# oscarknagg/voicemap

Measured on AMD Instinct MI355X. Metric: audio-sec/s embedded, 3s@16kHz siamese batch (training step), higher is better.
Workload: dtype f16; 1 GPU; siamese cfg-A train step (filters 128, embed 64, contrastive loss), 128 pairs/GPU of 3 s @ 16 kHz decimated x4 (L=12000), Adam(clipnorm 1), f16 storage; global_pairs=128, parallelism=dp1

## Files before the change

voicemap_amd/csrc/conv_common.hpp:

```cpp
#pragma once
#include <string.h>

#include <type_traits>

#include "common.hpp"

namespace vm {

constexpr int BM = 128, BN = 128;

template <int KB>
struct Geo {
    static constexpr int PITCH = KB + 16;
    static constexpr int TILE = BM * PITCH;
    static constexpr int CH = KB / 16;
    static constexpr int NCHUNK = BM * CH / 256;
};
constexpr int OUT_PITCH = BN * 4 + 16;

template <typename T> struct Mfma;
template <> struct Mfma<bf16> {
    static constexpr int KSTEP_BYTES = 32;
    using Frag = bf16x8;
    __device__ static inline Frag load(const char* row_ptr, int s, int kh) {
        return *reinterpret_cast<const Frag*>(row_ptr + (s * 2 + kh) * 16);
    }
    __device__ static inline f32x16 run(Frag a, Frag b, f32x16 c) {
        return __builtin_amdgcn_mfma_f32_32x32x16_bf16(a, b, c, 0, 0, 0);
    }
};
template <> struct Mfma<f16> {
    static constexpr int KSTEP_BYTES = 32;
    using Frag = f16x8;
    __device__ static inline Frag load(const char* row_ptr, int s, int kh) {
        return *reinterpret_cast<const Frag*>(row_ptr + (s * 2 + kh) * 16);
    }
    __device__ static inline f32x16 run(Frag a, Frag b, f32x16 c) {
        return __builtin_amdgcn_mfma_f32_32x32x16_f16(a, b, c, 0, 0, 0);
    }
};
template <> struct Mfma<float> {
    static constexpr int KSTEP_BYTES = 8;
    using Frag = float;
    __device__ static inline Frag load(const char* row_ptr, int s, int kh) {
        return *reinterpret_cast<const float*>(row_ptr + (s * 2 + kh) * 4);
    }
    __device__ static inline f32x16 run(Frag a, Frag b, f32x16 c) {
        return __builtin_amdgcn_mfma_f32_32x32x2f32(a, b, c, 0, 0, 0);
    }
};

template <typename T>
__device__ inline typename Mfma<T>::Frag ones16() {
    static_assert(sizeof(T) == 2, "16-bit storage types only");
    const uint32_t w = std::is_same<T, bf16>::value ? 0x3F803F80u : 0x3C003C00u;
    const u32x4 v = {w, w, w, w};
    return __builtin_bit_cast(typename Mfma<T>::Frag, v);
}

template <typename T> struct Mfma4;
template <> struct Mfma4<f16> {
// ... 159 lines not shown
```

voicemap_amd/csrc/conv_gemm.hip:

```cpp
#include "conv_common.hpp"

#ifndef VM_ABL
#define VM_ABL 0
#endif

namespace vm {

template <int KB>
constexpr int nt_lds_bytes() {
    return (2 * 2 * Geo<KB>::TILE > BM * OUT_PITCH + 4096) ? 2 * 2 * Geo<KB>::TILE : BM * OUT_PITCH + 4096;
}

template <typename T, int EPI, int KB, bool SPLIT = false>
__global__ __launch_bounds__(256) void conv_nt_kernel(NtArgs<T> p, int64_t n_groups) {
    static_assert(!SPLIT || (sizeof(T) == 4 && KB == 128), "split-bf16 arithmetic: fp32 storage, 128-byte slices");
    using G = Geo<KB>;
    constexpr int VEC = Elem<T>::kVec;
    constexpr int BK = KB / (int)sizeof(T);
    __shared__ __attribute__((aligned(16))) char lds[nt_lds_bytes<KB>()];

    const int tid = threadIdx.x, lane = tid & 63, w = tid >> 6, wm = w >> 1, wn = w & 1;
    const int nk = (p.Ktot + BK - 1) / BK;

    int lds_off[G::NCHUNK], kch[G::NCHUNK], srow[G::NCHUNK];
// ... 358 lines not shown
            issue(0);
            for (int kt = 0; kt < nk; ++kt) {
                __syncthreads();
                if (kt + 1 < nk) issue(kt + 1);
                const char* bufbase = lds + (kt & 1) * 2 * OPB;
                mma_slice_swz<T, KB>(bufbase, bufbase + OPB, wm, wn, lane, acc);
            }

            nt_epilogue<T, EPI>(p, lds, acc, n, tl, t0, n0, tid, lane, w, wm, wn);
            __syncthreads();
        }
    }
}

namespace n2 {
constexpr int TM = 256, TN = 128, KB = 64, RING = 3;
constexpr int A_BYTES = TM * KB, B_BYTES = TN * KB, STAGE = A_BYTES + B_BYTES;
constexpr int TP = TN * 2 + 16;
constexpr int LDS_BYTES = (RING * STAGE > TM * TP) ? RING * STAGE : TM * TP;
static_assert(2 * LDS_BYTES <= 160 * 1024, "two workgroups per CU");
}

template <typename T, int EPI>
__device__ inline void n2_load_bias(const NtArgs<T>& p, f32x4 (&b4)[2][4], int c0) {
#pragma unroll
    for (int j = 0; j < 2; ++j)
#pragma unroll
        for (int g = 0; g < 4; ++g) {
            b4[j][g] = f32x4{0.f, 0.f, 0.f, 0.f};
            if (EPI != EPI_DGRAD) b4[j][g] = *reinterpret_cast<const f32x4*>(p.bias + c0 + 32 * j + 8 * g);
        }
}
template <typename T>
__device__ inline void n2_fold_edge(const NtArgs<T>& p, f32x16 (&acc)[4][2], int row, int which, int wm, int r, int c0) {
    if ((row >> 7) != wm) return;
    const float* hb = p.fold_hb + (which ? 2 * p.N : 0) + c0;
    f32x4 h[2][4];
#pragma unroll
    for (int j = 0; j < 2; ++j)
#pragma unroll
        for (int g = 0; g < 4; ++g) h[j][g] = *reinterpret_cast<const f32x4*>(hb + 32 * j + 8 * g);
    const int rw = row & 127;
#pragma unroll
    for (int i = 0; i < 4; ++i) {
#pragma unroll
        for (int j = 0; j < 2; ++j) {
            const float m = (32 * i + r == rw) ? 1.f : 0.f;
#pragma unroll
            for (int g = 0; g < 4; ++g)
#pragma unroll
                for (int e = 0; e < 4; ++e) acc[i][j][4 * g + e] -= m * h[j][g][e];
        }
    }
}
__device__ inline void n2_fill_acc(f32x16 (&acc)[4][2], const f32x4 (&b4)[2][4]) {
#pragma unroll
    for (int j = 0; j < 2; ++j)
#pragma unroll
        for (int g = 0; g < 4; ++g)
#pragma unroll
            for (int i = 0; i < 4; ++i)
#pragma unroll
                for (int e = 0; e < 4; ++e) acc[i][j][4 * g + e] = b4[j][g][e];
}
#if defined(VM_EXPERIMENT_PROFILE_EPI)
extern __device__ unsigned int g_prof[];
__device__ inline void vm_epi_mark(int k) {
    const long long t = __builtin_amdgcn_s_memtime();
    if ((threadIdx.x & 63) == 0 && blockIdx.x < 8192) g_prof[((int64_t)blockIdx.x * 4 + (threadIdx.x >> 6)) * 8 + k] = (unsigned int)t;
}
#if VM_EXPERIMENT_PROFILE_EPI + 0 == 2
#define VM_EPI_MARK(k)
#define VM_RED_MARK(k) vm_epi_mark(k)
#else
#define VM_EPI_MARK(k) vm_epi_mark(k)
#define VM_RED_MARK(k)
#endif
#else
#define VM_EPI_MARK(k)
#define VM_RED_MARK(k)
#endif
struct N2DrainSync {
    __device__ inline void sync() { __syncthreads(); }
    __device__ inline void point() {}
};

template <typename T, int EPI>
__device__ inline void n2_tile_write(const NtArgs<T>& p, char* lds, const f32x16 (&acc)[4][2], int t0, int n0, int trows, int lane, int wm, int wn,
                                     const f32x4 (&negc)[2][4]) {
    using namespace n2;
    const int r = lane & 31, kh = lane >> 5;
    constexpr bool FWD = EPI == EPI_FWD || EPI == EPI_FWD_FOLD;
    const bool red = EPI == EPI_DGRAD && p.red_a != nullptr;
    const int valid = (p.L - t0) < trows ? (p.L - t0) : trows;
    constexpr bool CAN_CENTRE = EPI == EPI_FWD_FOLD && std::is_same<T, f16>::value;
    const bool ctrd = CAN_CENTRE && p.fold_ctr != nullptr;
    auto body = [&](auto ctrd_c) {
        constexpr bool CTRD = decltype(ctrd_c)::value;
        uint32_t nc16[2][4][2];
        if constexpr (CTRD) {
            typedef _Float16 h2 __attribute__((ext_vector_type(2)));
#pragma unroll
            for (int j = 0; j < 2; ++j)
#pragma unroll
                for (int g = 0; g < 4; ++g) {
                    nc16[j][g][0] = __builtin_bit_cast(uint32_t, h2{(_Float16)negc[j][g][0], (_Float16)negc[j][g][1]});
                    nc16[j][g][1] = __builtin_bit_cast(uint32_t, h2{(_Float16)negc[j][g][2], (_Float16)negc[j][g][3]});
                }
        }
#pragma unroll
        for (int i = 0; i < 4; ++i) {
#pragma unroll
            for (int j = 0; j < 2; ++j) {
                const int mb = wm * 128 + i * 32;
                const int m = mb + r;
                const bool partial = mb + 32 > valid;
                const bool zero = (FWD || red) && partial && m >= valid;
#pragma unroll
                for (int g = 0; g < 4; ++g) {
                    const int nl = wn * 64 + j * 32 + 8 * g + 4 * kh;
                    T o[4];
#pragma unroll
                    for (int e = 0; e < 4; ++e) o[e] = Elem<T>::from_f(acc[i][j][4 * g + e]);
                    u32x2 pk = *reinterpret_cast<const u32x2*>(o);
                    if constexpr (CTRD) {
                        uint32_t lo = pk[0], hi = pk[1];
                        asm("v_pk_max_f16 %0, %1, %2" : "=v"(lo) : "v"(lo), "v"(nc16[j][g][0]));
                        asm("v_pk_max_f16 %0, %1, %2" : "=v"(hi) : "v"(hi), "v"(nc16[j][g][1]));
                        pk[0] = lo;
                        pk[1] = hi;
                    } else if constexpr (EPI != EPI_DGRAD) {
                        uint32_t lo = pk[0], hi = pk[1];
                        asm("v_pk_max_i16 %0, %1, 0" : "=v"(lo) : "v"(lo));
                        asm("v_pk_max_i16 %0, %1, 0" : "=v"(hi) : "v"(hi));
                        pk[0] = lo;
                        pk[1] = hi;
                    }
                    pk[0] = zero ? 0u : pk[0];
                    pk[1] = zero ? 0u : pk[1];
                    *reinterpret_cast<u32x2*>(lds + m * TP + nl * 2) = pk;
                }
            }
        }
    };
    if constexpr (CAN_CENTRE) {
        if (ctrd) body(std::true_type{});
        else body(std::false_type{});
    } else {
        body(std::false_type{});
    }
}

template <typename T, int EPI, typename BarT>
__device__ inline void n2_tile_drain(const NtArgs<T>& p, char* lds, int64_t n, int tl, int t0, int n0, int trows, int tid, int lane, int w,
                                     BarT& bar) {
    using namespace n2;
    using V8 = typename Mfma<T>::Frag;
    const int kh = lane >> 5;
    constexpr bool FWD = EPI == EPI_FWD || EPI == EPI_FWD_FOLD;
    const bool stats = FWD && p.stat_sum != nullptr && !(VM_ABL & 8);
    const bool red = EPI == EPI_DGRAD && p.red_a != nullptr;
    const int valid = (p.L - t0) < trows ? (p.L - t0) : trows;
    const int c8 = tid & 15, rg = tid >> 4;
    if (EPI == EPI_FWD_POOL) {
// ... 283 lines not shown
                d2[h][1] = Mfma4<T>::run(dhi[q], ahi[rs], d2[h][1]);
            }
        }
        const int cn = lane & 31;
        const int rows2 = 2 * p.tilesL;
#pragma unroll
        for (int h = 0; h < 2; ++h) {
            float ds = d1[h][0][0] + d1[h][1][0], dq = 0.f;
#pragma unroll
            for (int e = 0; e < 4; ++e) dq = e == (lane & 3) ? d2[h][0][e] + d2[h][1][e] : dq;
            ds += __shfl_xor(ds, 32, 64);
            dq += __shfl_xor(dq, 32, 64);
            const int64_t srow = n * rows2 + 2 * tl + h;
            if (kh == 0) {
                p.stat_sum[srow * p.N + n0 + 32 * w + cn] = ds;
                p.stat_sq[srow * p.N + n0 + 32 * w + cn] = dq;
            }
        }
    }
}


template <typename T, int EPI>
__device__ inline void n2_epilogue(const NtArgs<T>& p, char* lds, const f32x16 (&acc)[4][2], int64_t n, int tl, int t0, int n0, int trows,
                                   int tid, int lane, int w, int wm, int wn) {
    f32x4 negc[2][4];
    if constexpr (EPI == EPI_FWD_FOLD && std::is_same<T, f16>::value) {
        if (p.fold_ctr != nullptr) {
#pragma unroll
            for (int j = 0; j < 2; ++j)
#pragma unroll
                for (int g = 0; g < 4; ++g) {
                    const f32x4 c = *reinterpret_cast<const f32x4*>(p.fold_ctr + n0 + (wn * 64 + j * 32) + 8 * g + 4 * (lane >> 5));
                    negc[j][g] = f32x4{-c[0], -c[1], -c[2], -c[3]};
                }
        }
    }
    VM_EPI_MARK(1);
    __syncthreads();
    VM_EPI_MARK(2);
    n2_tile_write<T, EPI>(p, lds, acc, t0, n0, trows, lane, wm, wn, negc);
    VM_EPI_MARK(3);
    __syncthreads();
    VM_EPI_MARK(4);
    N2DrainSync bar;
    n2_tile_drain<T, EPI>(p, lds, n, tl, t0, n0, trows, tid, lane, w, bar);
}

namespace n2r {
constexpr int TROWS = 254;
constexpr int A_BLK = 256 * 64, B_STG = 128 * 64;
constexpr int B0 = 3 * A_BLK;
constexpr int OPER = 3 * A_BLK + 3 * B_STG;
static_assert(OPER <= n2::LDS_BYTES, "operand rings fit under the epilogue tile");
}

__device__ inline void wait_vm_0246(int n) {
    if (n >= 6) {
// ... 49 lines not shown
    int tn;
    {
        const unsigned v = blockIdx.x, tiles_n = (unsigned)p.tilesN;
        if ((n_groups & 7) == 0) {
            const unsigned j = v >> 3, q = j / tiles_n;
            tn = (int)(j - q * tiles_n);
            group = q * 8 + (v & 7);
        } else {
            group = v / tiles_n;
            tn = (int)(v - group * tiles_n);
        }
    }
    const unsigned nw = group / (unsigned)p.tilesL;
    const int tl = (int)(group - nw * (unsigned)p.tilesL);
    const int64_t n = nw;
    const int t0 = tl * TROWS, n0 = tn * TN;
    if (n2_pool_dead_tile<T, EPI>(p, n, t0, n0, tid)) return;
    if constexpr (EPI == EPI_FWD_FOLD) {
        const unsigned tw = nw / (unsigned)p.tower_windows;
        p.bt += tw * p.bt_tower_stride;
        p.fold_hb += tw * 4 * p.N;
        if (p.fold_ctr != nullptr) p.fold_ctr += tw * p.N;
    }
    f32x4 bias4[2][4];
    if constexpr (EPI == EPI_FWD_FOLD) p.bias = p.fold_hb + 3 * p.N;
    n2_load_bias<T, EPI>(p, bias4, n0 + wn * 64 + 4 * (lane >> 5));

    const int lrow = lane >> 2, lchunk = lane & 3;
    const char* a_src[4];
    const char* b_src[2];
#pragma unroll
    for (int i = 0; i < 4; ++i) {
        const int row = (w + 4 * i) * 16 + lrow;
        int pr = t0 + row;
        pr = pr < p.L + 2 ? pr : p.L + 1;
        a_src[i] = reinterpret_cast<const char*>(p.a + n * p.a_win_stride + (int64_t)pr * p.a_c) + ((lchunk ^ ((row >> 2) & 3)) << 4);
    }
#pragma unroll
    for (int i = 0; i < 2; ++i) {
        const int row = (w + 4 * i) * 16 + lrow;
        b_src[i] = reinterpret_cast<const char*>(p.bt + (int64_t)(n0 + row) * p.Ktot) + ((lchunk ^ ((row >> 2) & 3)) << 4);
    }
    auto issue_a = [&](int blk, int chunk, int i0) {
        char* base = lds + blk * A_BLK;
#pragma unroll
        for (int i = 0; i < 2; ++i) glds16(a_src[i0 + i] + chunk * KB, base + __builtin_amdgcn_readfirstlane((w + 4 * (i0 + i)) * 1024));
    };
    auto issue_b = [&](int stg, int ko) {
        char* base = lds + B0 + stg * B_STG;
#pragma unroll
        for (int i = 0; i < 2; ++i) glds16(b_src[i] + ko, base + __builtin_amdgcn_readfirstlane((w + 4 * i) * 1024));
    };

    const int r = lane & 31, kh = lane >> 5;
    int a_addr[3][2], b_addr[2];
#pragma unroll
    for (int tap = 0; tap < 3; ++tap) {
        const int row = wm * 128 + r + tap;
#pragma unroll
        for (int ks = 0; ks < 2; ++ks) a_addr[tap][ks] = row * KB + (((2 * ks + kh) ^ ((row >> 2) & 3)) << 4);
    }
    {
        const int row = wn * 64 + r;
#pragma unroll
        for (int ks = 0; ks < 2; ++ks) b_addr[ks] = B0 + row * KB + (((2 * ks + kh) ^ ((row >> 2) & 3)) << 4);
    }

#if defined(__HIP_DEVICE_COMPILE__)
    const uint32_t lds0 = (uint32_t)(uintptr_t)(__attribute__((address_space(3))) const char*)lds;
#else
    const uint32_t lds0 = 0;
#endif

    VM_PROF(const long long pt_s2 = __builtin_amdgcn_s_memtime();)
    issue_a(0, 0, 0);
    issue_a(0, 0, 2);
    issue_b(0, 0);
    if (chunks > 1) {
        issue_a(1, 1, 0);
        issue_a(1, 1, 2);
    }
    issue_b(1, row_bytes);
    VM_PROF(const long long pt_s3 = __builtin_amdgcn_s_memtime();)
    f32x16 acc[4][2];
    n2_fill_acc(acc, bias4);
    int n_wait = (chunks > 1 ? 4 : 0) + 2;
    int ia_prev = 0;
    int b_tap = 2, b_chunk_off = 0, b_stage = 2;
    int a_blk = 0, b_cur = 0;
    for (int c = 0; c < chunks; ++c) {
        const bool more_a = c + 2 < chunks;
        const int a_next_blk = a_blk == 0 ? 2 : a_blk - 1;
#pragma unroll
        for (int tap = 0; tap < 3; ++tap) {
            const int kt = 3 * c + tap;
            wait_vm_0246(n_wait);
            __builtin_amdgcn_s_barrier();
            VM_PROF(if (kt == 0) pt_bar = __builtin_amdgcn_s_memtime();)
            int ib = 0, ia = 0;
            {
                if (kt + 2 < nk && !(VM_ABL & 1)) {
                    issue_b(b_stage, b_tap * row_bytes + b_chunk_off);
                    b_stage = b_stage == 2 ? 0 : b_stage + 1;
                    if (++b_tap == 3) {
                        b_tap = 0;
                        b_chunk_off += KB;
                    }
                    ib = 2;
                }
                if (tap < 2 && more_a && !(VM_ABL & 2)) {
                    issue_a(a_next_blk, c + 2, 2 * tap);
                    ia = 2;
                }
            }
            n_wait = ia_prev + ib + ia;
            ia_prev = ia;
            const uint32_t aa0 = lds0 + a_blk * A_BLK + a_addr[tap][0], aa1 = lds0 + a_blk * A_BLK + a_addr[tap][1];
            const uint32_t bb0 = lds0 + b_cur * B_STG + b_addr[0], bb1 = lds0 + b_cur * B_STG + b_addr[1];
            b_cur = b_cur == 2 ? 0 : b_cur + 1;
            u32x4 a0[4], b0[2], a1[4], b1[2];
            asm volatile("ds_read_b128 %0, %1" : "=v"(b0[0]) : "v"(bb0));
            asm volatile("ds_read_b128 %0, %1" : "=v"(a0[0]) : "v"(aa0));
            asm volatile("ds_read_b128 %0, %1 offset:2048" : "=v"(b0[1]) : "v"(bb0));
            asm volatile("ds_read_b128 %0, %1 offset:2048" : "=v"(a0[1]) : "v"(aa0));
            asm volatile("ds_read_b128 %0, %1 offset:4096" : "=v"(a0[2]) : "v"(aa0));
            asm volatile("ds_read_b128 %0, %1 offset:6144" : "=v"(a0[3]) : "v"(aa0));
            asm volatile("ds_read_b128 %0, %1" : "=v"(b1[0]) : "v"(bb1));
            asm volatile("ds_read_b128 %0, %1 offset:2048" : "=v"(b1[1]) : "v"(bb1));
            asm volatile("ds_read_b128 %0, %1" : "=v"(a1[0]) : "v"(aa1));
            asm volatile("ds_read_b128 %0, %1 offset:2048" : "=v"(a1[1]) : "v"(aa1));
            asm volatile("ds_read_b128 %0, %1 offset:4096" : "=v"(a1[2]) : "v"(aa1));
            asm volatile("ds_read_b128 %0, %1 offset:6144" : "=v"(a1[3]) : "v"(aa1));
#define VM_MM(A, B, I, J) acc[I][J] = Mfma<T>::run(__builtin_bit_cast(V8, B), __builtin_bit_cast(V8, A), acc[I][J])
            __builtin_amdgcn_sched_barrier(0);
            asm volatile("s_waitcnt lgkmcnt(9)" : "+v"(b0[0]), "+v"(a0[0]), "+v"(b0[1]));
            VM_MM(a0[0], b0[0], 0, 0);
            VM_MM(a0[0], b0[1], 0, 1);
            __builtin_amdgcn_sched_barrier(0);
            asm volatile("s_waitcnt lgkmcnt(8)" : "+v"(a0[1]));
            VM_MM(a0[1], b0[0], 1, 0);
            VM_MM(a0[1], b0[1], 1, 1);
            __builtin_amdgcn_sched_barrier(0);
            asm volatile("s_waitcnt lgkmcnt(7)" : "+v"(a0[2]));
            VM_MM(a0[2], b0[0], 2, 0);
            VM_MM(a0[2], b0[1], 2, 1);
            __builtin_amdgcn_sched_barrier(0);
            asm volatile("s_waitcnt lgkmcnt(6)" : "+v"(a0[3]));
            VM_MM(a0[3], b0[0], 3, 0);
            VM_MM(a0[3], b0[1], 3, 1);
            __builtin_amdgcn_sched_barrier(0);
            asm volatile("s_waitcnt lgkmcnt(3)" : "+v"(b1[0]), "+v"(b1[1]), "+v"(a1[0]));
            VM_MM(a1[0], b1[0], 0, 0);
            VM_MM(a1[0], b1[1], 0, 1);
            __builtin_amdgcn_sched_barrier(0);
            asm volatile("s_waitcnt lgkmcnt(2)" : "+v"(a1[1]));
            VM_MM(a1[1], b1[0], 1, 0);
            VM_MM(a1[1], b1[1], 1, 1);
            __builtin_amdgcn_sched_barrier(0);
            asm volatile("s_waitcnt lgkmcnt(1)" : "+v"(a1[2]));
            VM_MM(a1[2], b1[0], 2, 0);
            VM_MM(a1[2], b1[1], 2, 1);
            __builtin_amdgcn_sched_barrier(0);
            asm volatile("s_waitcnt lgkmcnt(0)" : "+v"(a1[3]));
            VM_MM(a1[3], b1[0], 3, 0);
            VM_MM(a1[3], b1[1], 3, 1);
            __builtin_amdgcn_sched_barrier(0);
#undef VM_MM
            __builtin_amdgcn_sched_barrier(0);
            VM_PROF(if (kt == 0) pt_first = __builtin_amdgcn_s_memtime();)
        }
        a_blk = a_blk == 2 ? 0 : a_blk + 1;
    }
    VM_PROF(const long long pt_loop = __builtin_amdgcn_s_memtime();)
    if constexpr (EPI == EPI_FWD_FOLD) {
        const int c0 = n0 + wn * 64 + 4 * (lane >> 5), rl = p.L - 1 - t0;
        if (t0 == 0) n2_fold_edge<T>(p, acc, 0, 0, wm, lane & 31, c0);
        if (rl >= 0 && rl < TROWS) n2_fold_edge<T>(p, acc, rl, 1, wm, lane & 31, c0);
    }
    n2_epilogue<T, EPI>(p, lds, acc, n, tl, t0, n0, TROWS, tid, lane, w, wm, wn);
#if defined(VM_EXPERIMENT_PROFILE)
    {
        asm volatile("s_waitcnt vmcnt(0)" ::: "memory");
        const long long pt_end = __builtin_amdgcn_s_memtime();
        if (lane == 0 && blockIdx.x < 8192) {
            unsigned int* q = g_prof + ((int64_t)blockIdx.x * 4 + w) * 8;
            q[0] = (unsigned int)(pt_end - pt_start);
            q[1] = (unsigned int)(pt_first - pt_start);
            q[2] = (unsigned int)(pt_loop - pt_first);
            q[3] = (unsigned int)(pt_end - pt_loop);
            q[4] = (unsigned int)(pt_s2 - pt_start);
            q[5] = (unsigned int)(pt_s3 - pt_s2);
            q[6] = (unsigned int)(pt_bar - pt_s3);
            q[7] = (unsigned int)(pt_first - pt_bar);
        }
    }
#endif
}


#ifndef VM_NT3_ABL
// ... 70 lines not shown
    {
        const unsigned v = blockIdx.x, tiles_n = (unsigned)p.tilesN;
        if ((n_groups & 7) == 0) {
            const unsigned j = v >> 3, q = j / tiles_n;
            tn = (int)(j - q * tiles_n);
            group = q * 8 + (v & 7);
        } else {
            group = v / tiles_n;
            tn = (int)(v - group * tiles_n);
        }
    }
    const unsigned nw = group / (unsigned)p.tilesL;
    const int tl = (int)(group - nw * (unsigned)p.tilesL);
    const int64_t n = nw;
    const int t0 = tl * n2r::TROWS, n0 = tn * TN;
    if (n2_pool_dead_tile<T, EPI>(p, n, t0, n0, tid)) return;
    unsigned tw = 0;
    if constexpr (EPI == EPI_FWD_FOLD) {
        tw = nw / (unsigned)p.tower_windows;
        p.fold_hb += tw * 4 * p.N;
        if (p.fold_ctr != nullptr) p.fold_ctr += tw * p.N;
    }
    if constexpr (EPI == EPI_FWD_FOLD) p.bias = p.fold_hb + 3 * p.N;
    f32x4 bias_lo[2][4], bias_hi[2][4];
    if constexpr (EPI != EPI_DGRAD) {
        const float* bp = p.bias + n0 + wn * 64;
#pragma unroll
        for (int j = 0; j < 2; ++j)
#pragma unroll
            for (int g = 0; g < 4; ++g) {
                bias_lo[j][g] = *reinterpret_cast<const f32x4*>(bp + 32 * j + 8 * g);
                bias_hi[j][g] = *reinterpret_cast<const f32x4*>(bp + 32 * j + 8 * g + 4);
            }
    }

    const int lrow = lane >> 2, lchunk = lane & 3;
    const char* a_src[4];
#pragma unroll
    for (int i = 0; i < 4; ++i) {
        const int row = (w + 4 * i) * 16 + lrow;
        int pr = t0 + row;
        pr = pr < p.L + 2 ? pr : p.L + 1;
        a_src[i] = reinterpret_cast<const char*>(p.a + n * p.a_win_stride + (int64_t)pr * p.a_c) + ((lchunk ^ ((row >> 2) & 3)) << 4);
    }
    auto issue_a = [&](int blk, int chunk, int i0) {
        char* base = lds + blk * A_BLK;
#pragma unroll
        for (int i = 0; i < 2; ++i) glds16(a_src[i0 + i] + chunk * KB, base + __builtin_amdgcn_readfirstlane((w + 4 * (i0 + i)) * 1024));
    };
    auto issue_a1 = [&](int blk, int chunk, int i) {
        glds16(a_src[i] + chunk * KB, lds + blk * A_BLK + __builtin_amdgcn_readfirstlane((w + 4 * i) * 1024));
    };
    uint64_t bbase;
    {
        const uint64_t q = (uint64_t)(uintptr_t)p.bt_packed +
                           ((uint64_t)tw * (unsigned)(p.N >> 6) + (unsigned)((n0 >> 6) + wn)) * (uint64_t)(NK * n3::KT_BYTES);
        const uint32_t lo = __builtin_amdgcn_readfirstlane((uint32_t)q), hi = __builtin_amdgcn_readfirstlane((uint32_t)(q >> 32));
        bbase = ((uint64_t)hi << 32) | lo;
    }
    const uint32_t bvoff = lane * 16;
    u32x4 bs[3][4];
#define VM_LOAD_SET(KT)                                                           \
    {                                                                             \
        const uint64_t sb_ = bbase + (uint64_t)((KT) * n3::KT_BYTES);             \
        VM_GLOAD_FRAG(bs[(KT) % 3][0], bvoff, sb_, 0);                            \
        VM_GLOAD_FRAG(bs[(KT) % 3][1], bvoff, sb_, 1024);                         \
        VM_GLOAD_FRAG(bs[(KT) % 3][2], bvoff, sb_, 2048);                         \
        VM_GLOAD_FRAG(bs[(KT) % 3][3], bvoff, sb_, 3072);                         \
    }

    const int r = lane & 31, kh = lane >> 5;
    int a_addr[3][2];
#pragma unroll
    for (int tap = 0; tap < 3; ++tap) {
        const int row = wm * 128 + r + tap;
#pragma unroll
        for (int ks = 0; ks < 2; ++ks) a_addr[tap][ks] = row * KB + (((2 * ks + kh) ^ ((row >> 2) & 3)) << 4);
    }
#if defined(__HIP_DEVICE_COMPILE__)
    const uint32_t lds0 = (uint32_t)(uintptr_t)(__attribute__((address_space(3))) const char*)lds;
#else
    const uint32_t lds0 = 0;
#endif

    VM_PROF(const long long pt_s2 = __builtin_amdgcn_s_memtime();)
    issue_a(0, 0, 0);
    issue_a(0, 0, 2);
    VM_LOAD_SET(0);
    if constexpr (LEAN) VM_LOAD_SET(1);
    if constexpr (CHUNKS > 1) {
        issue_a(1, 1, 0);
        issue_a(1, 1, 2);
    }
    if constexpr (!LEAN) {
        VM_LOAD_SET(1);
        if constexpr (CHUNKS > 2) {
            issue_a(2, 2, 0);
            issue_a(2, 2, 2);
        }
    }
    VM_PROF(const long long pt_s3 = __builtin_amdgcn_s_memtime();)
    f32x16 acc[4][2];
    {
        f32x4 bias4[2][4];
#pragma unroll
        for (int j = 0; j < 2; ++j)
#pragma unroll
            for (int g = 0; g < 4; ++g) {
                bias4[j][g] = f32x4{0.f, 0.f, 0.f, 0.f};
                if constexpr (EPI != EPI_DGRAD) bias4[j][g] = (lane >> 5) ? bias_hi[j][g] : bias_lo[j][g];
            }
        n2_fill_acc(acc, bias4);
    }
#if VM_NT3_ABL & 4
#define VM_MM(A, B, I, J) asm volatile("" : "+v"(acc[I][J]) : "v"(A), "v"(B))
#else
#define VM_MM(A, B, I, J) acc[I][J] = Mfma<T>::run(__builtin_bit_cast(V8, B), __builtin_bit_cast(V8, A), acc[I][J])
#endif
    u32x4 f0[4], f1[4];
#define VM_FRAG_READ(dst, base, I)                                                              \
    if constexpr ((I) == 0) asm volatile("ds_read_b128 %0, %1" : "=v"(dst) : "v"(base));          \
    if constexpr ((I) == 1) asm volatile("ds_read_b128 %0, %1 offset:2048" : "=v"(dst) : "v"(base)); \
    if constexpr ((I) == 2) asm volatile("ds_read_b128 %0, %1 offset:4096" : "=v"(dst) : "v"(base)); \
    if constexpr ((I) == 3) asm volatile("ds_read_b128 %0, %1 offset:6144" : "=v"(dst) : "v"(base));
#define VM_P_STEP0(I)                                                                                                                 \
    asm volatile("s_waitcnt lgkmcnt(3)" : "+v"(f0[I]));                                                                               \
    VM_MM(f0[I], bs[cur_][0], I, 0);                                                                                                  \
    VM_MM(f0[I], bs[cur_][2], I, 1);                                                                                                  \
    VM_FRAG_READ(f1[I], aa1_, I)                                                                                                      \
    if constexpr (kt_ + 2 < NK && !(VM_NT3_ABL & 1)) {                                                                                \
        if constexpr ((I) == 0) VM_GLOAD_FRAG(bs[nxt_][0], bvoff, sb_, 0);                                                            \
        if constexpr ((I) == 1) VM_GLOAD_FRAG(bs[nxt_][1], bvoff, sb_, 1024);                                                         \
        if constexpr ((I) == 2) VM_GLOAD_FRAG(bs[nxt_][2], bvoff, sb_, 2048);                                                         \
        if constexpr ((I) == 3) VM_GLOAD_FRAG(bs[nxt_][3], bvoff, sb_, 3072);                                                         \
    }                                                                                                                                 \
    __builtin_amdgcn_sched_barrier(0);
#define VM_P_STEP1(I)                                                                                                                 \
    if constexpr (kt_ + 1 < NK) {                                                                                                     \
        asm volatile("s_waitcnt lgkmcnt(3)" : "+v"(f1[I]));                                                                           \
    } else {                                                                                                                          \
        if constexpr ((I) == 0) asm volatile("s_waitcnt lgkmcnt(3)" : "+v"(f1[I]));                                                   \
        if constexpr ((I) == 1) asm volatile("s_waitcnt lgkmcnt(2)" : "+v"(f1[I]));                                                   \
        if constexpr ((I) == 2) asm volatile("s_waitcnt lgkmcnt(1)" : "+v"(f1[I]));                                                   \
        if constexpr ((I) == 3) asm volatile("s_waitcnt lgkmcnt(0)" : "+v"(f1[I]));                                                   \
    }                                                                                                                                 \
    VM_MM(f1[I], bs[cur_][1], I, 0);                                                                                                  \
    VM_MM(f1[I], bs[cur_][3], I, 1);                                                                                                  \
    if constexpr (kt_ + 1 < NK) { VM_FRAG_READ(f0[I], an0_, I) }                                                                      \
    if constexpr ((I) < n3_pieces(kt_, CHUNKS, LEAN).count && !(VM_NT3_ABL & 2))                                                      \
        issue_a1(n3_pieces(kt_, CHUNKS, LEAN).block % 4, n3_pieces(kt_, CHUNKS, LEAN).block, n3_pieces(kt_, CHUNKS, LEAN).first + (I)); \
    __builtin_amdgcn_sched_barrier(0);
#define VM_KTILE_P(KT)                                                                                                                \
    if constexpr ((KT) < NK) {                                                                                                        \
        constexpr int kt_ = (KT), c_ = kt_ / 3, tap_ = kt_ - 3 * c_, cur_ = kt_ % 3, nxt_ = (kt_ + 2) % 3, ablk_ = c_ % 4;             \
        constexpr int nc_ = (kt_ + 1) / 3, ntap_ = (kt_ + 1) - 3 * nc_;                             \
        n3_wait_b<n3_nwait(kt_, CHUNKS, LEAN)>(bs[cur_]);                                                                             \
        if constexpr (kt_ == 0) {                                                                                                     \
            __builtin_amdgcn_s_barrier();                                                                                             \
            VM_PROF(pt_bar = __builtin_amdgcn_s_memtime();)                                                                           \
            const uint32_t a00_ = lds0 + a_addr[0][0];                                                                                \
            VM_FRAG_READ(f0[0], a00_, 0) VM_FRAG_READ(f0[1], a00_, 1) VM_FRAG_READ(f0[2], a00_, 2) VM_FRAG_READ(f0[3], a00_, 3)         \
        }                                                                                                                             \
        const uint32_t aa1_ = lds0 + ablk_ * A_BLK + a_addr[tap_][1];                                                                  \
        const uint32_t an0_ = lds0 + (nc_ % 4) * A_BLK + a_addr[ntap_][0];                                                             \
        const uint64_t sb_ = bbase + (uint64_t)((kt_ + 2) * n3::KT_BYTES);                                                            \
        __builtin_amdgcn_sched_barrier(0);                                                                                            \
        VM_P_STEP0(0) VM_P_STEP0(1) VM_P_STEP0(2) VM_P_STEP0(3)                                                                       \
        if constexpr (tap_ == 2 && kt_ + 1 < NK) {                                                                                    \
            asm volatile("s_waitcnt lgkmcnt(0)" : "+v"(f1[0]), "+v"(f1[1]), "+v"(f1[2]), "+v"(f1[3]));                                 \
            __builtin_amdgcn_s_barrier();                                                                                             \
            __builtin_amdgcn_sched_barrier(0);                                                                                        \
        }                                                                                                                             \
        VM_P_STEP1(0) VM_P_STEP1(1) VM_P_STEP1(2) VM_P_STEP1(3)                                                                       \
        VM_PROF(if (kt_ == 0) pt_first = __builtin_amdgcn_s_memtime();)                                                               \
    }
#define VM_CHUNK(C) VM_KTILE_P(3 * (C)) VM_KTILE_P(3 * (C) + 1) VM_KTILE_P(3 * (C) + 2)
    VM_CHUNK(0) VM_CHUNK(1) VM_CHUNK(2) VM_CHUNK(3) VM_CHUNK(4) VM_CHUNK(5) VM_CHUNK(6) VM_CHUNK(7)
    VM_CHUNK(8) VM_CHUNK(9) VM_CHUNK(10) VM_CHUNK(11) VM_CHUNK(12) VM_CHUNK(13) VM_CHUNK(14) VM_CHUNK(15)
    static_assert(CHUNKS <= 16, "conv_nt3_kernel: at most 16 channel chunks are written out");
#undef VM_CHUNK
#undef VM_KTILE_P
#undef VM_P_STEP0
#undef VM_P_STEP1
#undef VM_FRAG_READ
#undef VM_MM
#undef VM_LOAD_SET
    if constexpr (EPI == EPI_FWD_FOLD) {
        const int c0 = n0 + wn * 64 + 4 * (lane >> 5), rl = p.L - 1 - t0;
        if (t0 == 0) n2_fold_edge<T>(p, acc, 0, 0, wm, lane & 31, c0);
        if (rl >= 0 && rl < n2r::TROWS) n2_fold_edge<T>(p, acc, rl, 1, wm, lane & 31, c0);
    }
    VM_PROF(const long long pt_loop = __builtin_amdgcn_s_memtime();)
#if VM_NT3_ABL & 8
    if (acc[0][0][0] == 123.456f && acc[3][1][15] == 1.5f) n2_epilogue<T, EPI>(p, lds, acc, n, tl, t0, n0, n2r::TROWS, tid, lane, w, wm, wn);
#else
    n2_epilogue<T, EPI>(p, lds, acc, n, tl, t0, n0, n2r::TROWS, tid, lane, w, wm, wn);
#endif
#if defined(VM_EXPERIMENT_PROFILE)
    {
        asm volatile("s_waitcnt vmcnt(0)" ::: "memory");
        const long long pt_end = __builtin_amdgcn_s_memtime();
#if defined(VM_EXPERIMENT_PROFILE_HW)
        if (lane == 0 && blockIdx.x < 8192) {
            unsigned int* q = g_prof + ((int64_t)blockIdx.x * 4 + w) * 8;
            q[0] = (unsigned int)pt_start;
            q[1] = (unsigned int)pt_end;
            q[2] = __builtin_amdgcn_s_getreg((31 << 11) | 4);
            q[3] = __builtin_amdgcn_s_getreg((31 << 11) | 20);
            q[4] = (unsigned int)pt_bar;
            q[5] = (unsigned int)pt_loop;
            q[6] = (unsigned int)(pt_start >> 32);
            q[7] = (unsigned int)pt_s3;
        }
        (void)pt_first; (void)pt_s2;
#elif defined(VM_EXPERIMENT_PROFILE_EPI)
        if (lane == 0 && blockIdx.x < 8192) {
            unsigned int* q = g_prof + ((int64_t)blockIdx.x * 4 + w) * 8;
// ... 486 lines not shown
```

Baseline: 296,700 audio-s/s.

## Switch n2/n3 conv GEMM inner loops from 32x32x16 to 16x16x32 MFMA tiles

Replaces the 32x32x16 MFMA instruction in the n2 and n3 conv kernels with 16x16x32 MFMA. Accumulators are reorganised from 4x2 f32x16 into 8x4 f32x4 fragments, with matching changes to the LDS read addressing, the B fragment global offsets, the bias fill and the epilogue writes. Each LDS read now covers the full K step, so fewer reads are issued per MFMA and the waits are interleaved row by row. The cost is that MFMA and layout indexing change throughout, which risks correctness and a different instruction-level schedule.

```diff
diff --git a/voicemap_amd/csrc/conv_common.hpp b/voicemap_amd/csrc/conv_common.hpp
--- a/voicemap_amd/csrc/conv_common.hpp
+++ b/voicemap_amd/csrc/conv_common.hpp
@@ -28,6 +28,9 @@
     __device__ static inline f32x16 run(Frag a, Frag b, f32x16 c) {
         return __builtin_amdgcn_mfma_f32_32x32x16_bf16(a, b, c, 0, 0, 0);
     }
+    __device__ static inline f32x4 run16(Frag a, Frag b, f32x4 c) {
+        return __builtin_amdgcn_mfma_f32_16x16x32_bf16(a, b, c, 0, 0, 0);
+    }
 };
 template <> struct Mfma<f16> {
     static constexpr int KSTEP_BYTES = 32;
@@ -37,6 +40,9 @@
     }
     __device__ static inline f32x16 run(Frag a, Frag b, f32x16 c) {
         return __builtin_amdgcn_mfma_f32_32x32x16_f16(a, b, c, 0, 0, 0);
+    }
+    __device__ static inline f32x4 run16(Frag a, Frag b, f32x4 c) {
+        return __builtin_amdgcn_mfma_f32_16x16x32_f16(a, b, c, 0, 0, 0);
     }
 };
 template <> struct Mfma<float> {
diff --git a/voicemap_amd/csrc/conv_gemm.hip b/voicemap_amd/csrc/conv_gemm.hip
--- a/voicemap_amd/csrc/conv_gemm.hip
+++ b/voicemap_amd/csrc/conv_gemm.hip
@@ -404,46 +404,35 @@
 }
 
 template <typename T, int EPI>
-__device__ inline void n2_load_bias(const NtArgs<T>& p, f32x4 (&b4)[2][4], int c0) {
-#pragma unroll
-    for (int j = 0; j < 2; ++j)
-#pragma unroll
-        for (int g = 0; g < 4; ++g) {
-            b4[j][g] = f32x4{0.f, 0.f, 0.f, 0.f};
-            if (EPI != EPI_DGRAD) b4[j][g] = *reinterpret_cast<const f32x4*>(p.bias + c0 + 32 * j + 8 * g);
-        }
+__device__ inline void n2_load_bias(const NtArgs<T>& p, f32x4 (&b4)[4], int c0) {
+#pragma unroll
+    for (int j = 0; j < 4; ++j) {
+        b4[j] = f32x4{0.f, 0.f, 0.f, 0.f};
+        if (EPI != EPI_DGRAD) b4[j] = *reinterpret_cast<const f32x4*>(p.bias + c0 + 16 * j);
+    }
 }
 template <typename T>
-__device__ inline void n2_fold_edge(const NtArgs<T>& p, f32x16 (&acc)[4][2], int row, int which, int wm, int r, int c0) {
+__device__ inline void n2_fold_edge(const NtArgs<T>& p, f32x4 (&acc)[8][4], int row, int which, int wm, int r, int c0) {
     if ((row >> 7) != wm) return;
     const float* hb = p.fold_hb + (which ? 2 * p.N : 0) + c0;
-    f32x4 h[2][4];
-#pragma unroll
-    for (int j = 0; j < 2; ++j)
-#pragma unroll
-        for (int g = 0; g < 4; ++g) h[j][g] = *reinterpret_cast<const f32x4*>(hb + 32 * j + 8 * g);
+    f32x4 h[4];
+#pragma unroll
+    for (int j = 0; j < 4; ++j) h[j] = *reinterpret_cast<const f32x4*>(hb + 16 * j);
     const int rw = row & 127;
 #pragma unroll
-    for (int i = 0; i < 4; ++i) {
-#pragma unroll
-        for (int j = 0; j < 2; ++j) {
-            const float m = (32 * i + r == rw) ? 1.f : 0.f;
-#pragma unroll
-            for (int g = 0; g < 4; ++g)
-#pragma unroll
-                for (int e = 0; e < 4; ++e) acc[i][j][4 * g + e] -= m * h[j][g][e];
-        }
-    }
-}
-__device__ inline void n2_fill_acc(f32x16 (&acc)[4][2], const f32x4 (&b4)[2][4]) {
-#pragma unroll
-    for (int j = 0; j < 2; ++j)
-#pragma unroll
-        for (int g = 0; g < 4; ++g)
-#pragma unroll
-            for (int i = 0; i < 4; ++i)
-#pragma unroll
-                for (int e = 0; e < 4; ++e) acc[i][j][4 * g + e] = b4[j][g][e];
+    for (int i = 0; i < 8; ++i) {
+        const float m = (16 * i + r == rw) ? 1.f : 0.f;
+#pragma unroll
+        for (int j = 0; j < 4; ++j)
+#pragma unroll
+            for (int e = 0; e < 4; ++e) acc[i][j][e] -= m * h[j][e];
+    }
+}
+__device__ inline void n2_fill_acc(f32x4 (&acc)[8][4], const f32x4 (&b4)[4]) {
+#pragma unroll
+    for (int j = 0; j < 4; ++j)
+#pragma unroll
+        for (int i = 0; i < 8; ++i) acc[i][j] = b4[j];
 }
 #if defined(VM_EXPERIMENT_PROFILE_EPI)
 extern __device__ unsigned int g_prof[];
@@ -468,10 +457,10 @@
 };
 
 template <typename T, int EPI>
-__device__ inline void n2_tile_write(const NtArgs<T>& p, char* lds, const f32x16 (&acc)[4][2], int t0, int n0, int trows, int lane, int wm, int wn,
-                                     const f32x4 (&negc)[2][4]) {
+__device__ inline void n2_tile_write(const NtArgs<T>& p, char* lds, const f32x4 (&acc)[8][4], int t0, int n0, int trows, int lane, int wm, int wn,
+                                     const f32x4 (&negc)[4]) {
     using namespace n2;
-    const int r = lane & 31, kh = lane >> 5;
+    const int r = lane & 15, q = lane >> 4;
     constexpr bool FWD = EPI == EPI_FWD || EPI == EPI_FWD_FOLD;
     const bool red = EPI == EPI_DGRAD && p.red_a != nullptr;
     const int valid = (p.L - t0) < trows ? (p.L - t0) : trows;
@@ -479,49 +468,44 @@
     const bool ctrd = CAN_CENTRE && p.fold_ctr != nullptr;
     auto body = [&](auto ctrd_c) {
         constexpr bool CTRD = decltype(ctrd_c)::value;
-        uint32_t nc16[2][4][2];
+        uint32_t nc16[4][2];
         if constexpr (CTRD) {
             typedef _Float16 h2 __attribute__((ext_vector_type(2)));
 #pragma unroll
-            for (int j = 0; j < 2; ++j)
-#pragma unroll
-                for (int g = 0; g < 4; ++g) {
-                    nc16[j][g][0] = __builtin_bit_cast(uint32_t, h2{(_Float16)negc[j][g][0], (_Float16)negc[j][g][1]});
-                    nc16[j][g][1] = __builtin_bit_cast(uint32_t, h2{(_Float16)negc[j][g][2], (_Float16)negc[j][g][3]});
+            for (int j = 0; j < 4; ++j) {
+                nc16[j][0] = __builtin_bit_cast(uint32_t, h2{(_Float16)negc[j][0], (_Float16)negc[j][1]});
+                nc16[j][1] = __builtin_bit_cast(uint32_t, h2{(_Float16)negc[j][2], (_Float16)negc[j][3]});
+            }
+        }
+#pragma unroll
+        for (int i = 0; i < 8; ++i) {
+            const int mb = wm * 128 + i * 16;
+            const int m = mb + r;
+            const bool partial = mb + 16 > valid;
+            const bool zero = (FWD || red) && partial && m >= valid;
+#pragma unroll
+            for (int j = 0; j < 4; ++j) {
+                const int nl = wn * 64 + j * 16 + 4 * q;
+                T o[4];
+#pragma unroll
+                for (int e = 0; e < 4; ++e) o[e] = Elem<T>::from_f(acc[i][j][e]);
+                u32x2 pk = *reinterpret_cast<const u32x2*>(o);
+                if constexpr (CTRD) {
+                    uint32_t lo = pk[0], hi = pk[1];
+                    asm("v_pk_max_f16 %0, %1, %2" : "=v"(lo) : "v"(lo), "v"(nc16[j][0]));
+                    asm("v_pk_max_f16 %0, %1, %2" : "=v"(hi) : "v"(hi), "v"(nc16[j][1]));
+                    pk[0] = lo;
+                    pk[1] = hi;
+                } else if constexpr (EPI != EPI_DGRAD) {
+                    uint32_t lo = pk[0], hi = pk[1];
+                    asm("v_pk_max_i16 %0, %1, 0" : "=v"(lo) : "v"(lo));
+                    asm("v_pk_max_i16 %0, %1, 0" : "=v"(hi) : "v"(hi));
+                    pk[0] = lo;
+                    pk[1] = hi;
                 }
-        }
-#pragma unroll
-        for (int i = 0; i < 4; ++i) {
-#pragma unroll
-            for (int j = 0; j < 2; ++j) {
-                const int mb = wm * 128 + i * 32;
-                const int m = mb + r;
-                const bool partial = mb + 32 > valid;
-                const bool zero = (FWD || red) && partial && m >= valid;
-#pragma unroll
-                for (int g = 0; g < 4; ++g) {
-                    const int nl = wn * 64 + j * 32 + 8 * g + 4 * kh;
-                    T o[4];
-#pragma unroll
-                    for (int e = 0; e < 4; ++e) o[e] = Elem<T>::from_f(acc[i][j][4 * g + e]);
-                    u32x2 pk = *reinterpret_cast<const u32x2*>(o);
-                    if constexpr (CTRD) {
-                        uint32_t lo = pk[0], hi = pk[1];
-                        asm("v_pk_max_f16 %0, %1, %2" : "=v"(lo) : "v"(lo), "v"(nc16[j][g][0]));
-                        asm("v_pk_max_f16 %0, %1, %2" : "=v"(hi) : "v"(hi), "v"(nc16[j][g][1]));
-                        pk[0] = lo;
-                        pk[1] = hi;
-                    } else if constexpr (EPI != EPI_DGRAD) {
-                        uint32_t lo = pk[0], hi = pk[1];
-                        asm("v_pk_max_i16 %0, %1, 0" : "=v"(lo) : "v"(lo));
-                        asm("v_pk_max_i16 %0, %1, 0" : "=v"(hi) : "v"(hi));
-                        pk[0] = lo;
-                        pk[1] = hi;
-                    }
-                    pk[0] = zero ? 0u : pk[0];
-                    pk[1] = zero ? 0u : pk[1];
-                    *reinterpret_cast<u32x2*>(lds + m * TP + nl * 2) = pk;
-                }
+                pk[0] = zero ? 0u : pk[0];
+                pk[1] = zero ? 0u : pk[1];
+                *reinterpret_cast<u32x2*>(lds + m * TP + nl * 2) = pk;
             }
         }
     };
@@ -851,18 +835,16 @@
 
 
 template <typename T, int EPI>
-__device__ inline void n2_epilogue(const NtArgs<T>& p, char* lds, const f32x16 (&acc)[4][2], int64_t n, int tl, int t0, int n0, int trows,
+__device__ inline void n2_epilogue(const NtArgs<T>& p, char* lds, const f32x4 (&acc)[8][4], int64_t n, int tl, int t0, int n0, int trows,
                                    int tid, int lane, int w, int wm, int wn) {
-    f32x4 negc[2][4];
+    f32x4 negc[4];
     if constexpr (EPI == EPI_FWD_FOLD && std::is_same<T, f16>::value) {
         if (p.fold_ctr != nullptr) {
 #pragma unroll
-            for (int j = 0; j < 2; ++j)
-#pragma unroll
-                for (int g = 0; g < 4; ++g) {
-                    const f32x4 c = *reinterpret_cast<const f32x4*>(p.fold_ctr + n0 + (wn * 64 + j * 32) + 8 * g + 4 * (lane >> 5));
-                    negc[j][g] = f32x4{-c[0], -c[1], -c[2], -c[3]};
-                }
+            for (int j = 0; j < 4; ++j) {
+                const f32x4 c = *reinterpret_cast<const f32x4*>(p.fold_ctr + n0 + (wn * 64 + j * 16) + 4 * (lane >> 4));
+                negc[j] = f32x4{-c[0], -c[1], -c[2], -c[3]};
+            }
         }
     }
     VM_EPI_MARK(1);
@@ -958,9 +940,9 @@
         p.fold_hb += tw * 4 * p.N;
         if (p.fold_ctr != nullptr) p.fold_ctr += tw * p.N;
     }
-    f32x4 bias4[2][4];
+    f32x4 bias4[4];
     if constexpr (EPI == EPI_FWD_FOLD) p.bias = p.fold_hb + 3 * p.N;
-    n2_load_bias<T, EPI>(p, bias4, n0 + wn * 64 + 4 * (lane >> 5));
+    n2_load_bias<T, EPI>(p, bias4, n0 + wn * 64 + 4 * (lane >> 4));
 
     const int lrow = lane >> 2, lchunk = lane & 3;
     const char* a_src[4];
@@ -988,18 +970,16 @@
         for (int i = 0; i < 2; ++i) glds16(b_src[i] + ko, base + __builtin_amdgcn_readfirstlane((w + 4 * i) * 1024));
     };
 
-    const int r = lane & 31, kh = lane >> 5;
-    int a_addr[3][2], b_addr[2];
+    const int r = lane & 15, q = lane >> 4;
+    int a_addr[3], b_addr;
 #pragma unroll
     for (int tap = 0; tap < 3; ++tap) {
         const int row = wm * 128 + r + tap;
-#pragma unroll
-        for (int ks = 0; ks < 2; ++ks) a_addr[tap][ks] = row * KB + (((2 * ks + kh) ^ ((row >> 2) & 3)) << 4);
+        a_addr[tap] = row * KB + ((q ^ ((row >> 2) & 3)) << 4);
     }
     {
         const int row = wn * 64 + r;
-#pragma unroll
-        for (int ks = 0; ks < 2; ++ks) b_addr[ks] = B0 + row * KB + (((2 * ks + kh) ^ ((row >> 2) & 3)) << 4);
+        b_addr = B0 + row * KB + ((q ^ ((row >> 2) & 3)) << 4);
     }
 
 #if defined(__HIP_DEVICE_COMPILE__)
@@ -1018,7 +998,7 @@
     }
     issue_b(1, row_bytes);
     VM_PROF(const long long pt_s3 = __builtin_amdgcn_s_memtime();)
-    f32x16 acc[4][2];
+    f32x4 acc[8][4];
     n2_fill_acc(acc, bias4);
     int n_wait = (chunks > 1 ? 4 : 0) + 2;
     int ia_prev = 0;
@@ -1051,56 +1031,27 @@
             }
             n_wait = ia_prev + ib + ia;
             ia_prev = ia;
-            const uint32_t aa0 = lds0 + a_blk * A_BLK + a_addr[tap][0], aa1 = lds0 + a_blk * A_BLK + a_addr[tap][1];
-            const uint32_t bb0 = lds0 + b_cur * B_STG + b_addr[0], bb1 = lds0 + b_cur * B_STG + b_addr[1];
+            const uint32_t aa = lds0 + a_blk * A_BLK + a_addr[tap];
+            const uint32_t bb = lds0 + b_cur * B_STG + b_addr;
             b_cur = b_cur == 2 ? 0 : b_cur + 1;
-            u32x4 a0[4], b0[2], a1[4], b1[2];
-            asm volatile("ds_read_b128 %0, %1" : "=v"(b0[0]) : "v"(bb0));
-            asm volatile("ds_read_b128 %0, %1" : "=v"(a0[0]) : "v"(aa0));
-            asm volatile("ds_read_b128 %0, %1 offset:2048" : "=v"(b0[1]) : "v"(bb0));
-            asm volatile("ds_read_b128 %0, %1 offset:2048" : "=v"(a0[1]) : "v"(aa0));
-            asm volatile("ds_read_b128 %0, %1 offset:4096" : "=v"(a0[2]) : "v"(aa0));
-            asm volatile("ds_read_b128 %0, %1 offset:6144" : "=v"(a0[3]) : "v"(aa0));
-            asm volatile("ds_read_b128 %0, %1" : "=v"(b1[0]) : "v"(bb1));
-            asm volatile("ds_read_b128 %0, %1 offset:2048" : "=v"(b1[1]) : "v"(bb1));
-            asm volatile("ds_read_b128 %0, %1" : "=v"(a1[0]) : "v"(aa1));
-            asm volatile("ds_read_b128 %0, %1 offset:2048" : "=v"(a1[1]) : "v"(aa1));
-            asm volatile("ds_read_b128 %0, %1 offset:4096" : "=v"(a1[2]) : "v"(aa1));
-            asm volatile("ds_read_b128 %0, %1 offset:6144" : "=v"(a1[3]) : "v"(aa1));
-#define VM_MM(A, B, I, J) acc[I][J] = Mfma<T>::run(__builtin_bit_cast(V8, B), __builtin_bit_cast(V8, A), acc[I][J])
+            u32x4 fa[8], fb[4];
+#define VM_DSR(dst, base, I) asm volatile("ds_read_b128 %0, %1 offset:%2" : "=v"(dst) : "v"(base), "n"((I) * 1024))
+            VM_DSR(fb[0], bb, 0); VM_DSR(fb[1], bb, 1); VM_DSR(fb[2], bb, 2); VM_DSR(fb[3], bb, 3);
+            VM_DSR(fa[0], aa, 0); VM_DSR(fa[1], aa, 1); VM_DSR(fa[2], aa, 2); VM_DSR(fa[3], aa, 3);
+            VM_DSR(fa[4], aa, 4); VM_DSR(fa[5], aa, 5); VM_DSR(fa[6], aa, 6); VM_DSR(fa[7], aa, 7);
+#undef VM_DSR
+#define VM_MM(A, B, I, J) acc[I][J] = Mfma<T>::run16(__builtin_bit_cast(V8, B), __builtin_bit_cast(V8, A), acc[I][J])
+#define VM_ROW(I, N)                                                  \
+            asm volatile("s_waitcnt lgkmcnt(" #N ")" : "+v"(fa[I]));  \
+            VM_MM(fa[I], fb[0], I, 0);                                \
+            VM_MM(fa[I], fb[1], I, 1);                                \
+            VM_MM(fa[I], fb[2], I, 2);                                \
+            VM_MM(fa[I], fb[3], I, 3);                                \
             __builtin_amdgcn_sched_barrier(0);
-            asm volatile("s_waitcnt lgkmcnt(9)" : "+v"(b0[0]), "+v"(a0[0]), "+v"(b0[1]));
-            VM_MM(a0[0], b0[0], 0, 0);
-            VM_MM(a0[0], b0[1], 0, 1);
             __builtin_amdgcn_sched_barrier(0);
-            asm volatile("s_waitcnt lgkmcnt(8)" : "+v"(a0[1]));
-            VM_MM(a0[1], b0[0], 1, 0);
-            VM_MM(a0[1], b0[1], 1, 1);
-            __builtin_amdgcn_sched_barrier(0);
-            asm volatile("s_waitcnt lgkmcnt(7)" : "+v"(a0[2]));
-            VM_MM(a0[2], b0[0], 2, 0);
-            VM_MM(a0[2], b0[1], 2, 1);
-            __builtin_amdgcn_sched_barrier(0);
-            asm volatile("s_waitcnt lgkmcnt(6)" : "+v"(a0[3]));
-            VM_MM(a0[3], b0[0], 3, 0);
-            VM_MM(a0[3], b0[1], 3, 1);
-            __builtin_amdgcn_sched_barrier(0);
-            asm volatile("s_waitcnt lgkmcnt(3)" : "+v"(b1[0]), "+v"(b1[1]), "+v"(a1[0]));
-            VM_MM(a1[0], b1[0], 0, 0);
-            VM_MM(a1[0], b1[1], 0, 1);
-            __builtin_amdgcn_sched_barrier(0);
-            asm volatile("s_waitcnt lgkmcnt(2)" : "+v"(a1[1]));
-            VM_MM(a1[1], b1[0], 1, 0);
-            VM_MM(a1[1], b1[1], 1, 1);
-            __builtin_amdgcn_sched_barrier(0);
-            asm volatile("s_waitcnt lgkmcnt(1)" : "+v"(a1[2]));
-            VM_MM(a1[2], b1[0], 2, 0);
-            VM_MM(a1[2], b1[1], 2, 1);
-            __builtin_amdgcn_sched_barrier(0);
-            asm volatile("s_waitcnt lgkmcnt(0)" : "+v"(a1[3]));
-            VM_MM(a1[3], b1[0], 3, 0);
-            VM_MM(a1[3], b1[1], 3, 1);
-            __builtin_amdgcn_sched_barrier(0);
+            asm volatile("s_waitcnt lgkmcnt(8)" : "+v"(fb[0]), "+v"(fb[1]), "+v"(fb[2]), "+v"(fb[3]));
+            VM_ROW(0, 7) VM_ROW(1, 6) VM_ROW(2, 5) VM_ROW(3, 4) VM_ROW(4, 3) VM_ROW(5, 2) VM_ROW(6, 1) VM_ROW(7, 0)
+#undef VM_ROW
 #undef VM_MM
             __builtin_amdgcn_sched_barrier(0);
             VM_PROF(if (kt == 0) pt_first = __builtin_amdgcn_s_memtime();)
@@ -1109,9 +1060,9 @@
     }
     VM_PROF(const long long pt_loop = __builtin_amdgcn_s_memtime();)
     if constexpr (EPI == EPI_FWD_FOLD) {
-        const int c0 = n0 + wn * 64 + 4 * (lane >> 5), rl = p.L - 1 - t0;
-        if (t0 == 0) n2_fold_edge<T>(p, acc, 0, 0, wm, lane & 31, c0);
-        if (rl >= 0 && rl < TROWS) n2_fold_edge<T>(p, acc, rl, 1, wm, lane & 31, c0);
+        const int c0 = n0 + wn * 64 + 4 * (lane >> 4), rl = p.L - 1 - t0;
+        if (t0 == 0) n2_fold_edge<T>(p, acc, 0, 0, wm, lane & 15, c0);
+        if (rl >= 0 && rl < TROWS) n2_fold_edge<T>(p, acc, rl, 1, wm, lane & 15, c0);
     }
     n2_epilogue<T, EPI>(p, lds, acc, n, tl, t0, n0, TROWS, tid, lane, w, wm, wn);
 #if defined(VM_EXPERIMENT_PROFILE)
@@ -1228,16 +1179,11 @@
         if (p.fold_ctr != nullptr) p.fold_ctr += tw * p.N;
     }
     if constexpr (EPI == EPI_FWD_FOLD) p.bias = p.fold_hb + 3 * p.N;
-    f32x4 bias_lo[2][4], bias_hi[2][4];
+    f32x4 bias_w[16];
     if constexpr (EPI != EPI_DGRAD) {
         const float* bp = p.bias + n0 + wn * 64;
 #pragma unroll
-        for (int j = 0; j < 2; ++j)
-#pragma unroll
-            for (int g = 0; g < 4; ++g) {
-                bias_lo[j][g] = *reinterpret_cast<const f32x4*>(bp + 32 * j + 8 * g);
-                bias_hi[j][g] = *reinterpret_cast<const f32x4*>(bp + 32 * j + 8 * g + 4);
-            }
+        for (int k = 0; k < 16; ++k) bias_w[k] = *reinterpret_cast<const f32x4*>(bp + 4 * k);
     }
 
     const int lrow = lane >> 2, lchunk = lane & 3;
@@ -1264,24 +1210,23 @@
         const uint32_t lo = __builtin_amdgcn_readfirstlane((uint32_t)q), hi = __builtin_amdgcn_readfirstlane((uint32_t)(q >> 32));
         bbase = ((uint64_t)hi << 32) | lo;
     }
-    const uint32_t bvoff = lane * 16;
+    const int r = lane & 15, q = lane >> 4;
+    const uint32_t bvoff = (q >> 1) * 1024 + (q & 1) * 512 + r * 16;
     u32x4 bs[3][4];
 #define VM_LOAD_SET(KT)                                                           \
     {                                                                             \
         const uint64_t sb_ = bbase + (uint64_t)((KT) * n3::KT_BYTES);             \
         VM_GLOAD_FRAG(bs[(KT) % 3][0], bvoff, sb_, 0);                            \
-        VM_GLOAD_FRAG(bs[(KT) % 3][1], bvoff, sb_, 1024);                         \
+        VM_GLOAD_FRAG(bs[(KT) % 3][1], bvoff, sb_, 256);                          \
         VM_GLOAD_FRAG(bs[(KT) % 3][2], bvoff, sb_, 2048);                         \
-        VM_GLOAD_FRAG(bs[(KT) % 3][3], bvoff, sb_, 3072);                         \
-    }
-
-    const int r = lane & 31, kh = lane >> 5;
-    int a_addr[3][2];
+        VM_GLOAD_FRAG(bs[(KT) % 3][3], bvoff, sb_, 2304);                         \
+    }
+
+    int a_addr[3];
 #pragma unroll
     for (int tap = 0; tap < 3; ++tap) {
         const int row = wm * 128 + r + tap;
-#pragma unroll
-        for (int ks = 0; ks < 2; ++ks) a_addr[tap][ks] = row * KB + (((2 * ks + kh) ^ ((row >> 2) & 3)) << 4);
+        a_addr[tap] = row * KB + ((q ^ ((row >> 2) & 3)) << 4);
     }
 #if defined(__HIP_DEVICE_COMPILE__)
     const uint32_t lds0 = (uint32_t)(uintptr_t)(__attribute__((address_space(3))) const char*)lds;
@@ -1306,39 +1251,36 @@
         }
     }
     VM_PROF(const long long pt_s3 = __builtin_amdgcn_s_memtime();)
-    f32x16 acc[4][2];
+    f32x4 acc[8][4];
     {
-        f32x4 bias4[2][4];
-#pragma unroll
-        for (int j = 0; j < 2; ++j)
-#pragma unroll
-            for (int g = 0; g < 4; ++g) {
-                bias4[j][g] = f32x4{0.f, 0.f, 0.f, 0.f};
-                if constexpr (EPI != EPI_DGRAD) bias4[j][g] = (lane >> 5) ? bias_hi[j][g] : bias_lo[j][g];
-            }
+        f32x4 bias4[4];
+#pragma unroll
+        for (int j = 0; j < 4; ++j) {
+            bias4[j] = f32x4{0.f, 0.f, 0.f, 0.f};
+            if constexpr (EPI != EPI_DGRAD)
+                bias4[j] = q == 0 ? bias_w[4 * j] : q == 1 ? bias_w[4 * j + 1] : q == 2 ? bias_w[4 * j + 2] : bias_w[4 * j + 3];
+        }
         n2_fill_acc(acc, bias4);
     }
 #if VM_NT3_ABL & 4
 #define VM_MM(A, B, I, J) asm volatile("" : "+v"(acc[I][J]) : "v"(A), "v"(B))
 #else
-#define VM_MM(A, B, I, J) acc[I][J] = Mfma<T>::run(__builtin_bit_cast(V8, B), __builtin_bit_cast(V8, A), acc[I][J])
+#define VM_MM(A, B, I, J) acc[I][J] = Mfma<T>::run16(__builtin_bit_cast(V8, B), __builtin_bit_cast(V8, A), acc[I][J])
 #endif
     u32x4 f0[4], f1[4];
-#define VM_FRAG_READ(dst, base, I)                                                              \
-    if constexpr ((I) == 0) asm volatile("ds_read_b128 %0, %1" : "=v"(dst) : "v"(base));          \
-    if constexpr ((I) == 1) asm volatile("ds_read_b128 %0, %1 offset:2048" : "=v"(dst) : "v"(base)); \
-    if constexpr ((I) == 2) asm volatile("ds_read_b128 %0, %1 offset:4096" : "=v"(dst) : "v"(base)); \
-    if constexpr ((I) == 3) asm volatile("ds_read_b128 %0, %1 offset:6144" : "=v"(dst) : "v"(base));
+#define VM_FRAG_READ(dst, base, B) asm volatile("ds_read_b128 %0, %1 offset:%2" : "=v"(dst) : "v"(base), "n"((B) * 1024));
 #define VM_P_STEP0(I)                                                                                                                 \
     asm volatile("s_waitcnt lgkmcnt(3)" : "+v"(f0[I]));                                                                               \
     VM_MM(f0[I], bs[cur_][0], I, 0);                                                                                                  \
-    VM_MM(f0[I], bs[cur_][2], I, 1);                                                                                                  \
-    VM_FRAG_READ(f1[I], aa1_, I)                                                                                                      \
+    VM_MM(f0[I], bs[cur_][1], I, 1);                                                                                                  \
+    VM_MM(f0[I], bs[cur_][2], I, 2);                                                                                                  \
+    VM_MM(f0[I], bs[cur_][3], I, 3);                                                                                                  \
+    VM_FRAG_READ(f1[I], aa_, 4 + (I))                                                                                                 \
     if constexpr (kt_ + 2 < NK && !(VM_NT3_ABL & 1)) {                                                                                \
         if constexpr ((I) == 0) VM_GLOAD_FRAG(bs[nxt_][0], bvoff, sb_, 0);                                                            \
-        if constexpr ((I) == 1) VM_GLOAD_FRAG(bs[nxt_][1], bvoff, sb_, 1024);                                                         \
+        if constexpr ((I) == 1) VM_GLOAD_FRAG(bs[nxt_][1], bvoff, sb_, 256);                                                          \
         if constexpr ((I) == 2) VM_GLOAD_FRAG(bs[nxt_][2], bvoff, sb_, 2048);                                                         \
-        if constexpr ((I) == 3) VM_GLOAD_FRAG(bs[nxt_][3], bvoff, sb_, 3072);                                                         \
+        if constexpr ((I) == 3) VM_GLOAD_FRAG(bs[nxt_][3], bvoff, sb_, 2304);                                                         \
     }                                                                                                                                 \
     __builtin_amdgcn_sched_barrier(0);
 #define VM_P_STEP1(I)                                                                                                                 \
@@ -1350,9 +1292,11 @@
         if constexpr ((I) == 2) asm volatile("s_waitcnt lgkmcnt(1)" : "+v"(f1[I]));                                                   \
         if constexpr ((I) == 3) asm volatile("s_waitcnt lgkmcnt(0)" : "+v"(f1[I]));                                                   \
     }                                                                                                                                 \
-    VM_MM(f1[I], bs[cur_][1], I, 0);                                                                                                  \
-    VM_MM(f1[I], bs[cur_][3], I, 1);                                                                                                  \
-    if constexpr (kt_ + 1 < NK) { VM_FRAG_READ(f0[I], an0_, I) }                                                                      \
+    VM_MM(f1[I], bs[cur_][0], 4 + (I), 0);                                                                                            \
+    VM_MM(f1[I], bs[cur_][1], 4 + (I), 1);                                                                                            \
+    VM_MM(f1[I], bs[cur_][2], 4 + (I), 2);                                                                                            \
+    VM_MM(f1[I], bs[cur_][3], 4 + (I), 3);                                                                                            \
+    if constexpr (kt_ + 1 < NK) { VM_FRAG_READ(f0[I], an_, I) }                                                                      \
     if constexpr ((I) < n3_pieces(kt_, CHUNKS, LEAN).count && !(VM_NT3_ABL & 2))                                                      \
         issue_a1(n3_pieces(kt_, CHUNKS, LEAN).block % 4, n3_pieces(kt_, CHUNKS, LEAN).block, n3_pieces(kt_, CHUNKS, LEAN).first + (I)); \
     __builtin_amdgcn_sched_barrier(0);
@@ -1364,11 +1308,11 @@
         if constexpr (kt_ == 0) {                                                                                                     \
             __builtin_amdgcn_s_barrier();                                                                                             \
             VM_PROF(pt_bar = __builtin_amdgcn_s_memtime();)                                                                           \
-            const uint32_t a00_ = lds0 + a_addr[0][0];                                                                                \
+            const uint32_t a00_ = lds0 + a_addr[0];                                                                                \
             VM_FRAG_READ(f0[0], a00_, 0) VM_FRAG_READ(f0[1], a00_, 1) VM_FRAG_READ(f0[2], a00_, 2) VM_FRAG_READ(f0[3], a00_, 3)         \
         }                                                                                                                             \
-        const uint32_t aa1_ = lds0 + ablk_ * A_BLK + a_addr[tap_][1];                                                                  \
-        const uint32_t an0_ = lds0 + (nc_ % 4) * A_BLK + a_addr[ntap_][0];                                                             \
+        const uint32_t aa_ = lds0 + ablk_ * A_BLK + a_addr[tap_];                                                                      \
+        const uint32_t an_ = lds0 + (nc_ % 4) * A_BLK + a_addr[ntap_];                                                                 \
         const uint64_t sb_ = bbase + (uint64_t)((kt_ + 2) * n3::KT_BYTES);                                                            \
         __builtin_amdgcn_sched_barrier(0);                                                                                            \
         VM_P_STEP0(0) VM_P_STEP0(1) VM_P_STEP0(2) VM_P_STEP0(3)                                                                       \
@@ -1392,13 +1336,13 @@
 #undef VM_MM
 #undef VM_LOAD_SET
     if constexpr (EPI == EPI_FWD_FOLD) {
-        const int c0 = n0 + wn * 64 + 4 * (lane >> 5), rl = p.L - 1 - t0;
-        if (t0 == 0) n2_fold_edge<T>(p, acc, 0, 0, wm, lane & 31, c0);
-        if (rl >= 0 && rl < n2r::TROWS) n2_fold_edge<T>(p, acc, rl, 1, wm, lane & 31, c0);
+        const int c0 = n0 + wn * 64 + 4 * q, rl = p.L - 1 - t0;
+        if (t0 == 0) n2_fold_edge<T>(p, acc, 0, 0, wm, r, c0);
+        if (rl >= 0 && rl < n2r::TROWS) n2_fold_edge<T>(p, acc, rl, 1, wm, r, c0);
     }
     VM_PROF(const long long pt_loop = __builtin_amdgcn_s_memtime();)
 #if VM_NT3_ABL & 8
-    if (acc[0][0][0] == 123.456f && acc[3][1][15] == 1.5f) n2_epilogue<T, EPI>(p, lds, acc, n, tl, t0, n0, n2r::TROWS, tid, lane, w, wm, wn);
+    if (acc[0][0][0] == 123.456f && acc[7][3][3] == 1.5f) n2_epilogue<T, EPI>(p, lds, acc, n, tl, t0, n0, n2r::TROWS, tid, lane, w, wm, wn);
 #else
     n2_epilogue<T, EPI>(p, lds, acc, n, tl, t0, n0, n2r::TROWS, tid, lane, w, wm, wn);
 #endif
```

Measured after the change: 303,200 audio-s/s, median of 6. 1.02x the previous value.
